# SerezD/vqvae-vqgan-pytorch-lightning

Measured on AMD Instinct MI355X. Metric: images/sec/node (256x256 bs=32/GPU) VQ-VAE train step, higher is better.
Workload: dtype bf16; 1 GPU; standard_vqvae cb=1024, 256x256 bs=32/GPU (encoder+VQ+decoder fwd/bwd + AdamW); yaml=example_confs/standard_vqvae.yaml, global_batch=32, parallelism=dp1, launch=hipGraph replay (fwd+bwd) + eager all-reduce + AdamW, deterministic=False

## Files before the change

### vqvae-vqgan-pytorch-lightning_amd/csrc/conv_mx.hip

```cpp
#include "conv_geom.h"
#include <stdlib.h>

namespace {
using vqkd::ConvGeom;
using vqkd::pack_bf16x2;
using vqkd::xcd_remap;

#ifndef VQK_MXABL
#define VQK_MXABL 0
#endif
#ifndef VQK_MX_RD
#define VQK_MX_RD 6
#endif
#ifndef VQK_MX_NT
#define VQK_MX_NT 2
#endif
#ifndef VQK_MX_HALO_AUX
#define VQK_MX_HALO_AUX 0
#endif
#ifndef VQK_MX_PRIO
#define VQK_MX_PRIO 0
#endif
#ifndef VQK_MX_PACE
#define VQK_MX_PACE 0
#endif
#ifndef VQK_MX_WL
#define VQK_MX_WL 0
#endif
#ifndef VQK_MX_JOUTER
#define VQK_MX_JOUTER 0
#endif
#ifndef VQK_MX_PIN
#define VQK_MX_PIN 1
#endif

#define SGB(mask, n) __builtin_amdgcn_sched_group_barrier(mask, n, 0)

__host__ __device__ constexpr int mx_tap_pix(bool s2, int tap, int twd, int hw2, int shp) {
    return s2 ? (((tap / 3) & 1) * 2 + ((tap % 3) & 1)) * shp + ((tap / 3) >> 1) * hw2 + ((tap % 3) >> 1)
              : (tap / twd) * hw2 + (tap % twd);
}

template <int TWLOG, bool POOL, int NTAP, int PIXELS = 256, int TAPW = 0, bool S2 = false>
__global__ __launch_bounds__(512, 2) void conv3x3_mx_kernel(const bf16_raw* __restrict__ x, const bf16_raw* __restrict__ wp,
                                                            const float* __restrict__ bias,
                                                            const bf16_raw* __restrict__ res, bf16_raw* __restrict__ y,
                                                            ConvGeom g) {
    constexpr int HM = NTAP == 1 ? 0 : 1;
    constexpr int PIX = PIXELS, TW = 1 << TWLOG, TH = PIX / TW;
    constexpr int HW2 = S2 ? TW + 1 : TW + 2 * HM;
    constexpr int SHP = (TH + 1) * (TW + 1);
    constexpr int HROWS = S2 ? 4 * SHP : (TH + 2 * HM) * HW2;
    constexpr int RS = 80;
    constexpr int PIECES = (HROWS * 5 + 63) / 64;
    constexpr int NBUF = S2 ? 2 : 3;
    constexpr int BUF = PIECES * 1024, STG = NBUF * BUF, SPITCH = 272, SCR = STG + PIX * SPITCH;
    constexpr int TQR = SCR + 1024;
    constexpr int TWD = TAPW ? TAPW : NTAP == 9 ? 3 : NTAP == 4 ? 2 : 1;
    constexpr int NI = VQK_MX_WL ? PIX / 32 : PIX / 64, NJ = VQK_MX_WL ? 1 : 2;
    constexpr int NQ = PIX / 16;
    static_assert(PIX == 256 || ((PIX == 128 || PIX == 64) && !POOL && NTAP == 9), "256-pixel tiles, or plain 128- / 64-pixel part tiles");
    constexpr int NPH = NTAP * 2;
    static_assert(NTAP == 9 || ((NTAP == 4 || NTAP == 2 || NTAP == 1) && !POOL), "3x3 taps, the 2x2 / 1x2 / 2x1 taps of a phase, or a 1x1 conv");
    static_assert(!S2 || (NTAP == 9 && !POOL && PIX == 128), "stride 2: 3x3 taps, 128-pixel tiles");
    static_assert(TAPW == 0 || (NTAP == 2 && (TAPW == 1 || TAPW == 2)), "TAPW names the orientation of a 2-tap window");
    constexpr int XS = (PIECES + 3) / 4;
    constexpr int OOB = (int)0x80000000;
    typedef bf16x8_t frag_t;
    typedef __attribute__((ext_vector_type(4))) unsigned int u32x4;
    typedef __attribute__((ext_vector_type(2))) unsigned int u32x2;
    extern __shared__ __attribute__((aligned(16))) char smem[];

    const int tid = threadIdx.x, lane = tid & 63;
    const int wave = __builtin_amdgcn_readfirstlane(tid >> 6);
    const int tiles_x = g.w >> TWLOG, tiles_y = g.h / TH;
    const int pmode = NTAP == 4 ? g.phase_mode : 0;
    const int total_tiles = g.n * tiles_y * tiles_x * g.tiles_n * (pmode == 1 ? 4 : 1);
    const int nch = g.cpt >> 2;
    const int nun = pmode == 2 ? 4 * nch : nch;
    const int grid = (int)gridDim.x, q8 = grid >> 3, r8 = grid & 7, xcd = (int)blockIdx.x & 7;
    const int cnt = q8 + (xcd < r8 ? 1 : 0);
    const int c0 = xcd < r8 ? xcd * (q8 + 1) : r8 * (q8 + 1) + (xcd - r8) * q8;
    const int vbid = c0 + ((int)blockIdx.x >> 3);
    if (vbid >= total_tiles) return;
    auto tile_of = [&](int k) -> int { const int j = k / cnt; return c0 + (k - j * cnt) + j * grid; };
    const int tqm = g.tq ? g.tq_mode : 0;
    volatile VQK_LDS int* const ring = (volatile VQK_LDS int*)(smem + TQR);
    auto next_id = [&](int j) -> int { return tqm ? __builtin_amdgcn_readfirstlane(ring[j & 7]) : vbid + j * grid; };
    const bool pro_sync = tqm == 2 || (tqm && nun < 4);

    struct TilePos { int img, py0, px0, nt, ph; };
    auto tile_pos = [&](int t) -> TilePos {
        TilePos tp;
        tp.nt = t % g.tiles_n; t /= g.tiles_n;
        tp.ph = 0;
        if (pmode == 1) { tp.ph = t & 3; t >>= 2; }
        const int txi = t % tiles_x; t /= tiles_x;
        const int tyi = t % tiles_y;
        tp.img = t / tiles_y; tp.py0 = tyi * TH; tp.px0 = txi * TW;
        return tp;
    };
    auto unit_barrier = [&]() { asm volatile("s_waitcnt lgkmcnt(0)\n\ts_barrier" ::: "memory"); };
    double* const gnws = (VQK_MXABL & 64) ? nullptr : g.gn_ws;
    unsigned long long* const dbg = (VQK_MXABL & 64) ? reinterpret_cast<unsigned long long*>(g.gn_ws) : nullptr;

    if (wave < 4) {
        if (VQK_MX_PRIO) __builtin_amdgcn_s_setprio(VQK_MX_PRIO);
        const int wm = VQK_MX_WL ? 0 : wave >> 1, wn = VQK_MX_WL ? wave : wave & 1;
        const int p = lane & 31, kg = lane >> 5;
        unsigned abase[NI], sbase[NI];
#pragma unroll
        for (int i = 0; i < NI; ++i) {
            int ty, tx;
            if (TWLOG == 5) { ty = wm * NI + i; tx = p; }
            else { ty = wm * 2 * NI + 2 * i + (p >> 4); tx = p & 15; }
            abase[i] = (unsigned)(((ty + (pmode ? 0 : g.tap_oy)) * HW2 + tx + (pmode ? 0 : g.tap_ox)) * RS + kg * 16);
            sbase[i] = (unsigned)(STG + (ty * TW + tx) * SPITCH + (wn * (32 * NJ) + 4 * kg) * 2);
        }
        const int lane16 = lane * 16;
        const int phase_bytes = (g.cout >> 5) * nch * (NPH * 1024);
        const __amdgpu_buffer_rsrc_t wsrd = __builtin_amdgcn_make_buffer_rsrc(
            const_cast<bf16_raw*>(wp), 0, phase_bytes * (pmode ? 4 : 1), 0x00020000);
        auto unit_ph = [&](int key, int c) -> int { return pmode == 2 ? c / nch : (key >> 16); };
        auto unit_w = [&](int key, int c, int j) -> int {
            const int ph = unit_ph(key, c), cc = pmode == 2 ? c - ph * nch : c;
            const int wph = (NTAP == 4 && g.phase_rev) ? 3 - ph : ph;
            return wph * phase_bytes + (((key & 0xffff) * 4 + wn * NJ + j) * nch + cc) * (NPH * 1024);
        };
        auto phase_off = [&](int ph) -> int {
            const int a = ph >> 1, b = ph & 1;
            return pmode == 1 ? (a * HW2 + b) * RS : pmode == 2 ? ((1 - a) * HW2 + (1 - b)) * RS : 0;
        };
        auto tile_nt = [&](int t) -> int {
            return (t % g.tiles_n) | (pmode == 1 ? ((t / g.tiles_n) & 3) << 16 : 0);
        };
        auto wload = [&](int soff) -> frag_t {
            return __builtin_bit_cast(frag_t, __builtin_amdgcn_raw_buffer_load_b128(wsrd, lane16, soff, 0));
        };

        constexpr int RD = NTAP == 9 ? VQK_MX_RD : NTAP == 4 ? 4 : 2;
        static_assert(NPH % RD == 0, "weight ring depth must divide the phases of a unit");
        f32x16 acc[NI][NJ];
        frag_t bw[RD][NJ];
        int wcur[NJ];
        if (pro_sync) unit_barrier();
        const int t_first = tqm == 2 ? __builtin_amdgcn_readfirstlane(ring[0]) : vbid;
        if (t_first >= total_tiles) return;
        int cur_nt = tile_nt(t_first);
#pragma unroll
        for (int j = 0; j < NJ; ++j) wcur[j] = unit_w(cur_nt, 0, j);
#pragma unroll
        for (int d = 0; d < RD; ++d)
#pragma unroll
            for (int j = 0; j < NJ; ++j) bw[d][j] = wload(wcur[j] + d * 1024);
        unit_barrier();

        int tj = 0, c = 0, bi = 0, t_next = 0;
        unsigned long long t_bar = 0, t_park = 0, n_units = 0, t_c0 = 0, t_cl = 0, t_top = 0;
        const unsigned long long t_begin = (VQK_MXABL & 64) ? __builtin_amdgcn_s_memtime() : 0;
        for (;;) {
            if (VQK_MXABL & 64) t_top = __builtin_amdgcn_s_memtime();
            if (c == nun - 2) t_next = next_id(tj + 1);
            const bool last_c = c == nun - 1, more = last_c && t_next < total_tiles;
            int nc = c + 1, nxt_nt = cur_nt;
            if (last_c) {
                if (more) { nc = 0; nxt_nt = tile_nt(t_next); }
                else nc = c;
            }
            int wnxt[NJ];
#pragma unroll
            for (int j = 0; j < NJ; ++j) wnxt[j] = unit_w(nxt_nt, nc, j);
            const char* lbase[NI];
#pragma unroll
            for (int i = 0; i < NI; ++i) lbase[i] = smem + bi * BUF + abase[i] + (NTAP == 4 ? phase_off(unit_ph(cur_nt, c)) : 0);

            frag_t a[2][NI];
#pragma unroll
            for (int i = 0; i < NI; ++i) a[0][i] = *reinterpret_cast<const frag_t*>(lbase[i]);
            __builtin_amdgcn_sched_barrier(0);
#pragma unroll
            for (int tap = 0; tap < NTAP; ++tap) {
                const int toff = mx_tap_pix(S2, tap, TWD, HW2, SHP) * RS;
#pragma unroll
                for (int ks = 0; ks < 2; ++ks) {
                    const bool reads = ks == 0 || tap < NTAP - 1;
                    const int ph = tap * 2 + ks;
                    if (ks == 0) {
#pragma unroll
                        for (int i = 0; i < NI; ++i) a[1][i] = *reinterpret_cast<const frag_t*>(lbase[i] + toff + 32);
                    } else if (tap < NTAP - 1) {
                        const int toff1 = mx_tap_pix(S2, tap + 1, TWD, HW2, SHP) * RS;
#pragma unroll
                        for (int i = 0; i < NI; ++i) a[0][i] = *reinterpret_cast<const frag_t*>(lbase[i] + toff1);
                    }
                    if (tap == 0 && ks == 0 && c == 0) {
                        const f32x16 zero = {0.f, 0.f, 0.f, 0.f, 0.f, 0.f, 0.f, 0.f, 0.f, 0.f, 0.f, 0.f, 0.f, 0.f, 0.f, 0.f};
#pragma unroll
                        for (int i = 0; i < NI; ++i)
#pragma unroll
                            for (int j = 0; j < NJ; ++j)
                                acc[i][j] = __builtin_amdgcn_mfma_f32_32x32x16_bf16(bw[ph % RD][j], a[ks][i], zero, 0, 0, 0);
                    } else if (VQK_MX_JOUTER) {
#pragma unroll
                        for (int j = 0; j < NJ; ++j)
#pragma unroll
                            for (int i = 0; i < NI; ++i)
                                acc[i][j] = __builtin_amdgcn_mfma_f32_32x32x16_bf16(bw[ph % RD][j], a[ks][i], acc[i][j], 0, 0, 0);
                    } else {
#pragma unroll
                        for (int i = 0; i < NI; ++i)
#pragma unroll
                            for (int j = 0; j < NJ; ++j)
                                acc[i][j] = __builtin_amdgcn_mfma_f32_32x32x16_bf16(bw[ph % RD][j], a[ks][i], acc[i][j], 0, 0, 0);
                    }
#pragma unroll
                    for (int j = 0; j < NJ; ++j) {
                        const int soff = (ph + RD >= NPH) ? wnxt[j] + (ph + RD - NPH) * 1024 : wcur[j] + (ph + RD) * 1024;
                        bw[ph % RD][j] = wload(((VQK_MXABL & 32) && g.n > 0 && wm == 1) ? (soff & 1023) : soff);
                    }
                    if (VQK_MX_PIN) {
                        if (reads) {
#pragma unroll
                            for (int i = 0; i < NI; ++i) { SGB(0x008, 1); SGB(0x100, 1); }
                            if constexpr (NI * NJ - NI > 0) SGB(0x008, NI * NJ - NI);
                        } else {
                            SGB(0x008, NI * NJ);
                        }
                        SGB(0x020, NJ);
                    }
                    __builtin_amdgcn_sched_barrier(0);
                }
            }
            const unsigned long long t_a = (VQK_MXABL & 64) ? __builtin_amdgcn_s_memtime() : 0;
            if (VQK_MXABL & 64) { if (c == 0) t_c0 += t_a - t_top; if (c == nun - 1) t_cl += t_a - t_top; }
            if (c == nun - 1 && !((VQK_MXABL & 4) && g.n > 0)) {
#pragma unroll
                for (int i = 0; i < NI; ++i)
#pragma unroll
                    for (int j = 0; j < NJ; ++j)
#pragma unroll
                        for (int rq = 0; rq < 4; ++rq) {
                            const u32x2 o = {pack_bf16x2(acc[i][j][4 * rq], acc[i][j][4 * rq + 1]),
                                             pack_bf16x2(acc[i][j][4 * rq + 2], acc[i][j][4 * rq + 3])};
                            *reinterpret_cast<u32x2*>(smem + sbase[i] + (j * 32 + 8 * rq) * 2) = o;
                        }
            }
            if (VQK_MXABL & 64) {
                asm volatile("s_waitcnt lgkmcnt(0)" ::: "memory");
                const unsigned long long t_b = __builtin_amdgcn_s_memtime();
                unit_barrier();
                const unsigned long long t_c = __builtin_amdgcn_s_memtime();
                t_park += t_b - t_a; t_bar += t_c - t_b; ++n_units;
            } else
            unit_barrier();
            if (last_c) { if (!more) break; ++tj; }
            cur_nt = nxt_nt; c = nc;
            bi = bi == NBUF - 1 ? 0 : bi + 1;
#pragma unroll
            for (int j = 0; j < NJ; ++j) wcur[j] = wnxt[j];
        }
        if ((VQK_MXABL & 64) && dbg && lane == 0) {
            unsigned long long* o = dbg + ((int64_t)blockIdx.x * 4 + wave) * 8;
            o[0] = __builtin_amdgcn_s_memtime() - t_begin; o[1] = t_bar; o[2] = t_park; o[3] = n_units;
            o[4] = t_c0; o[5] = t_cl; o[6] = (unsigned long long)nun; o[7] = 0;
        }
        return;
    }

    const int xt = tid - 256, xw = wave - 4;
    const __amdgpu_buffer_rsrc_t xsrd = __builtin_amdgcn_make_buffer_rsrc(
        const_cast<bf16_raw*>(x), 0, (int)((int64_t)g.n * g.h_in * g.w_in * g.cin * 2), 0x00020000);
    const int out_bytes = (int)((int64_t)g.n * g.dst_h * g.dst_w * g.cout * 2);
    const __amdgpu_buffer_rsrc_t rsrd = __builtin_amdgcn_make_buffer_rsrc(const_cast<bf16_raw*>(res), 0, res ? out_bytes : 0, 0x00020000);
    const __amdgpu_buffer_rsrc_t ysrd = __builtin_amdgcn_make_buffer_rsrc(y, 0, out_bytes >> (POOL ? 2 : 0), 0x00020000);

    int rel[XS], flg[XS];
#pragma unroll
    for (int sl = 0; sl < XS; ++sl) {
        const int s = (xw + 4 * sl) * 64 + lane;
        const int hp = s / 5, cp = s - hp * 5;
        if constexpr (S2) {
            const int sh = hp / SHP, q = hp - sh * SHP;
            const int hy = q / HW2, hx = q - hy * HW2, pa = sh >> 1, pb = sh & 1;
            rel[sl] = (((2 * hy + pa) * g.w_in + 2 * hx + pb) * g.cin + cp * 8) * 2;
            flg[sl] = (cp == 4 || hp >= HROWS || (pa && hy == TH) || (pb && hx == TW)) ? 16 : 0;
        } else {
            const int hy = hp / HW2, hx = hp - hy * HW2;
            rel[sl] = (((((hy - HM) * g.src_s) >> g.ups) * g.w_in + (((hx - HM) * g.src_s) >> g.ups)) * g.cin + cp * 8) * 2;
            flg[sl] = (HM && hy == 0 ? 1 : 0) | (HM && hy == TH + 1 ? 2 : 0) | (HM && hx == 0 ? 4 : 0) | (HM && hx == TW + 1 ? 8 : 0) |
                      ((cp == 4 || hp >= HROWS) ? 16 : 0);
        }
    }
    auto issue_halo = [&](const TilePos& tp, int cu, int bufi) {
        const int uph = pmode == 2 ? cu / nch : 0, c = pmode == 2 ? cu - uph * nch : cu;
        const int sa = pmode == 2 ? (uph >> 1) : g.src_a, sb = pmode == 2 ? (uph & 1) : g.src_b;
        const int base = (((tp.img * g.h_in + ((tp.py0 * g.src_s + sa) >> g.ups)) * g.w_in + ((tp.px0 * g.src_s + sb) >> g.ups)) * g.cin + c * 32) * 2;
        const int tb = S2 ? 16 : ((tp.py0 == 0 ? 1 : 0) | (tp.py0 + TH == g.h ? 2 : 0) | (tp.px0 == 0 ? 4 : 0) | (tp.px0 + TW == g.w ? 8 : 0) | 16);
#pragma unroll
        for (int sl = 0; sl < XS; ++sl) {
            if (xw + 4 * sl < PIECES) {
                const int off = (flg[sl] & tb) ? OOB : base + rel[sl];
                __builtin_amdgcn_raw_ptr_buffer_load_lds(
                    xsrd, (VQK_LDS void*)(smem + bufi * BUF + (xw + 4 * sl) * 1024), 16,
                    (VQK_MXABL & 8) ? (off & 0x8003fff0) : off, 0, 0, VQK_MX_HALO_AUX);
            }
        }
    };
    auto unpack8 = [&](const u32x4& r, float (&v)[8]) {
#pragma unroll
        for (int e = 0; e < 4; ++e) { v[2 * e] = __uint_as_float(r[e] << 16); v[2 * e + 1] = __uint_as_float(r[e] & 0xffff0000u); }
    };
    auto pack8 = [&](const float (&v)[8]) -> u32x4 {
        const u32x4 o = {pack_bf16x2(v[0], v[1]), pack_bf16x2(v[2], v[3]), pack_bf16x2(v[4], v[5]), pack_bf16x2(v[6], v[7])};
        return o;
    };
    const int slot = xt & 15;
    constexpr int NP = POOL ? 4 : NQ;
    constexpr int NR = NQ;
    struct OutPos { int pix0, ppix0, co, img, tile; };
    auto out_pos = [&](const TilePos& tp) -> OutPos {
        OutPos o;
        o.tile = (tp.py0 / TH) * tiles_x + (tp.px0 >> TWLOG) + (pmode == 1 ? tp.ph * tiles_y * tiles_x : 0);
        const int da = pmode == 1 ? (tp.ph >> 1) : g.dst_a, db = pmode == 1 ? (tp.ph & 1) : g.dst_b;
        o.pix0 = (tp.img * g.dst_h + tp.py0 * g.dst_s + da) * g.dst_w + tp.px0 * g.dst_s + db;
        o.ppix0 = (tp.img * (g.h >> 1) + (tp.py0 >> 1)) * (g.w >> 1) + (tp.px0 >> 1);
        o.co = tp.nt * 128 + slot * 8;
        o.img = tp.img;
        return o;
    };
    auto res_off = [&](const OutPos& o, int k) -> int {
        int ty, tx;
        if constexpr (!POOL) { const int pp = k * 16 + (xt >> 4); ty = pp >> TWLOG; tx = pp & (TW - 1); }
        else { const int opp = (k >> 2) * 16 + (xt >> 4); ty = 2 * (opp >> (TWLOG - 1)) + ((k >> 1) & 1); tx = 2 * (opp & (TW / 2 - 1)) + (k & 1); }
        return ((o.pix0 + (ty * g.dst_w + tx) * g.dst_s) * g.cout + o.co) * 2;
    };
    auto load_res = [&](const OutPos& o, u32x4 (&rv)[NR]) {
#pragma unroll
        for (int k = 0; k < NR; ++k)
            rv[k] = __builtin_bit_cast(u32x4, __builtin_amdgcn_raw_buffer_load_b128(rsrd, res_off(o, k), 0, 0));
    };
    int stat_idx = -1;
    auto flush_stats = [&]() {
        if (xw == 0) {
            float v = 0.f;
#pragma unroll
            for (int k = 0; k < 4; ++k) v += *reinterpret_cast<const float*>(smem + SCR + (k * 64 + lane) * 4);
            if (g.gn_part_nblk) {
                const int span = g.gn_cpg >> 3;
                if (span >= 2) v += __shfl_xor(v, 1, 64);
                if (span >= 4) v += __shfl_xor(v, 2, 64);
                if (stat_idx >= 0 && (span < 2 || (lane & (span - 1)) == 0)) gnws[stat_idx] = (double)v;
            } else if (stat_idx >= 0) {
                atomicAdd(gnws + stat_idx, (double)v);
            }
        }
    };
    float ga = 0.f, qa = 0.f, gb = 0.f, qb = 0.f;
    auto drain = [&](const OutPos& o, const u32x4 (&rv)[NR], int k0, int k1, bool first, bool last) {
        if (first) { ga = 0.f; qa = 0.f; gb = 0.f; qb = 0.f; }
        float bv[8] = {0.f, 0.f, 0.f, 0.f, 0.f, 0.f, 0.f, 0.f};
        if (bias) {
            const f32x4 b0 = *reinterpret_cast<const f32x4*>(bias + o.co), b1 = *reinterpret_cast<const f32x4*>(bias + o.co + 4);
#pragma unroll
            for (int e = 0; e < 4; ++e) { bv[e] = b0[e]; bv[4 + e] = b1[e]; }
        }
        const bool want_stats = gnws != nullptr;
        const unsigned ones2 = 0x3f803f80u;
        auto tally = [&](const u32x4& o) {
            const unsigned d0 = o[0], d1 = o[1], d2 = o[2], d3 = o[3];
            asm("v_dot2c_f32_bf16 %0, %4, %8\n\tv_dot2c_f32_bf16 %1, %4, %4\n\tv_dot2c_f32_bf16 %2, %6, %8\n\t"
                "v_dot2c_f32_bf16 %3, %6, %6\n\tv_dot2c_f32_bf16 %0, %5, %8\n\tv_dot2c_f32_bf16 %1, %5, %5\n\t"
                "v_dot2c_f32_bf16 %2, %7, %8\n\tv_dot2c_f32_bf16 %3, %7, %7\n\ts_nop 0"
                : "+v"(ga), "+v"(qa), "+v"(gb), "+v"(qb) : "v"(d0), "v"(d1), "v"(d2), "v"(d3), "v"(ones2));
        };
        auto settle = [&]() { asm volatile("s_nop 3" : "+v"(ga), "+v"(qa), "+v"(gb), "+v"(qb)); };
        u32x4 t[NQ];
        if constexpr (!POOL) {
#pragma unroll
            for (int k = 0; k < NQ; ++k) {
                if (k < k0 || k >= k1) continue;
                t[k] = *reinterpret_cast<const u32x4*>(smem + STG + (k * 16 + (xt >> 4)) * SPITCH + slot * 16);
            }
        } else {
#pragma unroll
            for (int k = 0; k < NQ; ++k) {
                if ((k >> 2) < k0 || (k >> 2) >= k1) continue;
                const int opp = (k >> 2) * 16 + (xt >> 4);
                const int ty = 2 * (opp >> (TWLOG - 1)) + ((k >> 1) & 1), tx = 2 * (opp & (TW / 2 - 1)) + (k & 1);
                t[k] = *reinterpret_cast<const u32x4*>(smem + STG + (ty * TW + tx) * SPITCH + slot * 16);
            }
        }
        __builtin_amdgcn_sched_barrier(0);
        if constexpr (!POOL) {
            if (!bias && !res && g.act == 0 && g.acc_scale == 1.0f && g.out_gain == 1.0f) {
#pragma unroll
                for (int k = 0; k < NP; ++k) {
                    if (k < k0 || k >= k1) continue;
                    __builtin_amdgcn_raw_buffer_store_b128(t[k], ysrd, res_off(o, k), 0, VQK_MX_NT);
                    if (want_stats) tally(t[k]);
                }
            } else {
                const bool general = g.act != 0 || g.acc_scale != 1.0f || g.out_gain != 1.0f;
                float abl_b[8] = {0.f, 0.f, 0.f, 0.f, 0.f, 0.f, 0.f, 0.f}, abl_g[8] = {0.f, 0.f, 0.f, 0.f, 0.f, 0.f, 0.f, 0.f};
#pragma unroll
                for (int k = 0; k < NP; ++k) {
                    if (k < k0 || k >= k1) continue;
                    float f[8], r[8];
                    unpack8(t[k], f);
                    unpack8(rv[k], r);
                    if ((VQK_MXABL & 16) && g.n > 0) {
#pragma unroll
                        for (int e = 0; e < 8; ++e) {
                            const float xh = __fmaf_rn(r[e], 1.3f, -0.13f);
                            const float u = __fmaf_rn(xh, 1.1f, 0.05f);
                            const float sg = __frcp_rn(1.0f + __expf(-u));
                            const float t = f[e] * (sg * (1.0f + u * (1.0f - sg)));
                            abl_b[e] += t;
                            abl_g[e] = __fmaf_rn(t, xh, abl_g[e]);
                        }
                    }
                    if (general) {
#pragma unroll
                        for (int e = 0; e < 8; ++e) {
                            float v = __fmaf_rn(f[e], g.acc_scale, bv[e]);
                            v = g.act == 2 ? fmaxf(v, 0.0f) : g.act == 3 ? fmaxf(v, 0.2f * v) : v;
                            f[e] = __fmaf_rn(v, g.out_gain, r[e]);
                        }
                    } else {
#pragma unroll
                        for (int e = 0; e < 8; ++e) f[e] = f[e] + bv[e] + r[e];
                    }
                    const u32x4 ov = pack8(f);
                    __builtin_amdgcn_raw_buffer_store_b128(ov, ysrd, res_off(o, k), 0, VQK_MX_NT);
                    if (want_stats) tally(ov);
                }
                if ((VQK_MXABL & 16) && g.n > 0) {
#pragma unroll
                    for (int e = 0; e < 8; ++e) { ga += abl_b[e]; qa += abl_g[e]; }
                }
            }
        } else {
#pragma unroll
            for (int k = 0; k < NP; ++k) {
                if (k < k0 || k >= k1) continue;
                const int opp = k * 16 + (xt >> 4);
                const int oty = opp >> (TWLOG - 1), otx = opp & (TW / 2 - 1);
                float s[8] = {0.f, 0.f, 0.f, 0.f, 0.f, 0.f, 0.f, 0.f};
#pragma unroll
                for (int d = 0; d < 4; ++d) {
                    float f[8], r[8];
                    unpack8(t[4 * k + d], f);
                    unpack8(rv[4 * k + d], r);
#pragma unroll
                    for (int e = 0; e < 8; ++e) s[e] += f[e] + r[e];
                }
#pragma unroll
                for (int e = 0; e < 8; ++e) s[e] = (s[e] + 4.0f * bv[e]) * g.pool_scale;
                const u32x4 ov = pack8(s);
                __builtin_amdgcn_raw_buffer_store_b128(ov, ysrd, ((o.ppix0 + oty * (g.w >> 1) + otx) * g.cout + o.co) * 2, 0, VQK_MX_NT);
                if (want_stats) tally(ov);
            }
        }
        if (want_stats && last) {
            settle();
            const bool split = g.gn_cpg == 4;
            if (!split) { ga += gb; qa += qb; }
            ga += __shfl_xor(ga, 16, 64); ga += __shfl_xor(ga, 32, 64);
            qa += __shfl_xor(qa, 16, 64); qa += __shfl_xor(qa, 32, 64);
            if (split) {
                gb += __shfl_xor(gb, 16, 64); gb += __shfl_xor(gb, 32, 64);
                qb += __shfl_xor(qb, 16, 64); qb += __shfl_xor(qb, 32, 64);
            }
            const int q = (xt >> 4) & 3;
            const float val = q == 0 ? ga : q == 1 ? qa : q == 2 ? gb : qb;
            *reinterpret_cast<float*>(smem + SCR + (xw * 64 + lane) * 4) = val;
            const int grp = (o.co + (q >> 1) * 4) / g.gn_cpg;
            const int gslot = o.img * (g.cout / g.gn_cpg) + grp;
            stat_idx = (split || q < 2) ? ((g.gn_part_nblk ? gslot * g.gn_part_nblk + g.gn_part_base + o.tile : gslot) * 2 + (q & 1)) : -1;
        }
    };

    int nissued = tqm == 2 ? 0 : 1, exhausted = 0, pend = 0, fv = 0;
    const int qbase = tqm == 2 ? 0 : cnt;
    auto fetch_issue = [&]() {
        if (lane == 0) fv = __hip_atomic_fetch_add(g.tq + xcd, 1, __ATOMIC_RELAXED, __HIP_MEMORY_SCOPE_AGENT);
        pend = 1;
    };
    auto fetch_land = [&]() {
        const int t = tile_of(__builtin_amdgcn_readfirstlane(fv) + qbase);
        if (lane == 0) ring[nissued & 7] = t;
        ++nissued; pend = 0;
        if (t >= total_tiles) exhausted = 1;
    };
    auto census = [&]() {
        if (tqm && xw == 0 && lane == 0) {
            const int old = __hip_atomic_fetch_add(g.tq + 8, 1, __ATOMIC_RELAXED, __HIP_MEMORY_SCOPE_AGENT);
            if (old == grid - 1) {
#pragma unroll
                for (int i = 0; i < 9; ++i) __hip_atomic_exchange(g.tq + i, 0, __ATOMIC_RELAXED, __HIP_MEMORY_SCOPE_AGENT);
            }
        }
    };
    if (tqm && xw == 0) {
        const int need = 3 / nun;
        while (nissued <= need && !exhausted) { fetch_issue(); fetch_land(); }
    }
    if (pro_sync) unit_barrier();
    const int t_first = tqm == 2 ? __builtin_amdgcn_readfirstlane(ring[0]) : vbid;
    if (t_first >= total_tiles) { census(); return; }

    int ltj = 0, lc = 0, lbuf = 0, lvalid = 1, lnew = 0;
    TilePos ltp = tile_pos(t_first);
    auto look = [&]() {
        if (lnew) {
            lnew = 0;
            if (lvalid) {
                const int t = next_id(ltj);
                lvalid = t < total_tiles;
                if (lvalid) ltp = tile_pos(t);
            }
        }
    };
    auto bump = [&]() {
        if (++lc == nun) { lc = 0; ++ltj; lnew = 1; }
        lbuf = lbuf == NBUF - 1 ? 0 : lbuf + 1;
    };
    issue_halo(ltp, lc, lbuf); bump();
    if constexpr (NBUF == 3) { look(); if (lvalid) issue_halo(ltp, lc, lbuf); bump(); }
    int tj = 0, c = 0;
    TilePos cur = tile_pos(t_first);
    OutPos done = out_pos(cur);
    int fu = 4 % nun, ford = 4 / nun;
    bool pending = false, flush = false;
    int dk = 0;
    u32x4 rv[NR];
#pragma unroll
    for (int k = 0; k < NR; ++k) rv[k] = u32x4{0u, 0u, 0u, 0u};
    asm volatile("s_waitcnt vmcnt(0)" ::: "memory");
    unit_barrier();

    for (;;) {
        asm volatile("s_waitcnt vmcnt(0)" ::: "memory");
        if (tqm && xw == 0) {
            if (pend) fetch_land();
            if (!exhausted && ford >= nissued) fetch_issue();
        }
        if (++fu == nun) { fu = 0; ++ford; }
        if constexpr (NBUF == 2) {
            look();
            if (lvalid) issue_halo(ltp, lc, lbuf);
            bump();
        }
        if (flush) { flush_stats(); flush = false; }
        if (pending && !((VQK_MXABL & 2) && g.n > 0)) {
            const int per = (VQK_MX_PACE && nun > 2) ? (NP + nun - 2) / (nun - 1) : NP;
            const int k1 = dk + per < NP ? dk + per : NP;
            drain(done, rv, dk, k1, dk == 0, k1 == NP);
            dk = k1;
            if (dk == NP) { pending = false; dk = 0; flush = gnws != nullptr; }
        }
        const bool last_c = c == nun - 1;
        int t_next = 0;
        if (last_c) {
            pending = true;
            done = out_pos(cur);
            if (res) load_res(done, rv);
            t_next = next_id(tj + 1);
        }
        if constexpr (NBUF == 3) {
            look();
            if (lvalid && !((VQK_MXABL & 1) && g.n > 0)) issue_halo(ltp, lc, lbuf);
            bump();
        } else {
            asm volatile("s_waitcnt vmcnt(0)" ::: "memory");
        }
        unit_barrier();
        if (last_c) {
            if (t_next >= total_tiles) break;
            c = 0; ++tj; cur = tile_pos(t_next);
        } else {
            ++c;
        }
    }
    if (flush) flush_stats();
    if (pending) {
        asm volatile("s_waitcnt vmcnt(0)" ::: "memory");
        drain(done, rv, dk, NP, dk == 0, true);
        if (gnws) {
            unit_barrier();
            flush_stats();
        }
    }
    census();
}

}

namespace vqkd {

namespace {
template <auto Kern>
int mx_launch(dim3 grid, int lds, hipStream_t st, const void* x, const void* w, const float* bias, const void* res, void* y,
              const ConvGeom& g) {
    static const hipError_t attr = hipFuncSetAttribute((const void*)Kern, hipFuncAttributeMaxDynamicSharedMemorySize, lds);
    if (attr != hipSuccess) return VQK_ERR_LAUNCH;
    hipLaunchKernelGGL(Kern, grid, dim3(512), lds, st, (const bf16_raw*)x, (const bf16_raw*)w, bias, (const bf16_raw*)res,
                       (bf16_raw*)y, g);
    return hipGetLastError() == hipSuccess ? VQK_OK : VQK_ERR_LAUNCH;
}

int device_cus() {
    static const int cus = [] {
        int dev = 0, n = 0;
        if (hipGetDevice(&dev) != hipSuccess ||
            hipDeviceGetAttribute(&n, hipDeviceAttributeMultiprocessorCount, dev) != hipSuccess || n <= 0) n = 256;
        return n;
    }();
    return cus;
}
}

int launch_conv3x3_mx(const void* x, const void* w, const float* bias, const void* res, void* y, const void* zeros,
                      const ConvGeom& g_in, int twlog, hipStream_t st) {
    (void)zeros;
    ConvGeom g = g_in;
    if (!g.dst_h) { g.dst_h = g.h * g.dst_s; g.dst_w = g.w * g.dst_s; }
    const int half_on = VQK_TUNE("MX_HALF", 1);
    const int half_hw = VQK_TUNE("MX_HALF_HW", 256);
    const bool half = half_on && g.h * g.w <= half_hw && !g.pool && g.ntap == 9 && (twlog == 4 ? (g.h % 8) == 0 : (g.h % 4) == 0);
    const int qmode = VQK_TUNE("MX_QUARTER", 1);
    const bool quarter = half && qmode && (g.tiles_n <= 2 || qmode >= 2) && (twlog == 4 ? (g.h % 4) == 0 : (g.h % 2) == 0);
    const int th = (quarter ? 64 : half ? 128 : 256) >> twlog;
    const int total = g.n * (g.h / th) * (g.w >> twlog) * g.tiles_n * ((g.ntap == 4 && g.phase_mode == 1) ? 4 : 1);
    int cus = device_cus() - VQK_TUNE("COMM_CUS", 0);
    if (cus < 1) cus = 1;
    const dim3 grid((unsigned)(total < cus ? total : cus));
    const int tqm = VQK_TUNE("TILE_QUEUE", 0);
    const DetState& tqs = tile_queue_state();
    auto set_queue = [&](int tiles, int blocks) {
        const bool on = tqm > 0 && tqs.ws != nullptr && tqs.bytes >= 64 && tiles > blocks && (g.cpt >> 2) >= 2;
        g.tq = on ? reinterpret_cast<int*>(tqs.ws) : nullptr;
        g.tq_mode = on ? (tqm >= 2 ? 2 : 1) : 0;
    };
    set_queue(total, (int)grid.x);
    constexpr int TQB = 64;
    constexpr int lds5 = 3 * (((256 / 32 + 2) * 34 * 5 + 63) / 64) * 1024 + 256 * 272 + 1024 + TQB;
    constexpr int lds4 = 3 * (((256 / 16 + 2) * 18 * 5 + 63) / 64) * 1024 + 256 * 272 + 1024 + TQB;
    constexpr int lds4h = 3 * (((128 / 16 + 2) * 18 * 5 + 63) / 64) * 1024 + 128 * 272 + 1024 + TQB;
    constexpr int lds5h = 3 * (((128 / 32 + 2) * 34 * 5 + 63) / 64) * 1024 + 128 * 272 + 1024 + TQB;
#define MXL(K, L) return mx_launch<K>(grid, L, st, x, w, bias, res, y, g)
    constexpr int lds4q = 3 * (((64 / 16 + 2) * 18 * 5 + 63) / 64) * 1024 + 64 * 272 + 1024 + TQB;
    constexpr int lds5q = 3 * (((64 / 32 + 2) * 34 * 5 + 63) / 64) * 1024 + 64 * 272 + 1024 + TQB;
    if (g.s2) {
        constexpr int lds5s = 2 * ((4 * (128 / 32 + 1) * 33 * 5 + 63) / 64) * 1024 + 128 * 272 + 1024 + TQB;
        constexpr int lds4s = 2 * ((4 * (128 / 16 + 1) * 17 * 5 + 63) / 64) * 1024 + 128 * 272 + 1024 + TQB;
        if (g.pool || g.ntap != 9 || (twlog == 4 ? (g.h % 8) : (g.h % 4)) != 0) return VQK_ERR_ARG;
        const int tot2 = g.n * (g.h / (128 >> twlog)) * (g.w >> twlog) * g.tiles_n;
        const dim3 grid2((unsigned)(tot2 < cus ? tot2 : cus));
        set_queue(tot2, (int)grid2.x);
        if (twlog == 5) return mx_launch<conv3x3_mx_kernel<5, false, 9, 128, 0, true>>(grid2, lds5s, st, x, w, bias, res, y, g);
        return mx_launch<conv3x3_mx_kernel<4, false, 9, 128, 0, true>>(grid2, lds4s, st, x, w, bias, res, y, g);
    }
    if (g.ntap == 2) {
        if (g.pool) return VQK_ERR_ARG;
        if (g.tapw == 2) { if (twlog == 5) MXL((conv3x3_mx_kernel<5, false, 2, 256, 2>), lds5); else MXL((conv3x3_mx_kernel<4, false, 2, 256, 2>), lds4); }
        if (g.tapw == 1) { if (twlog == 5) MXL((conv3x3_mx_kernel<5, false, 2, 256, 1>), lds5); else MXL((conv3x3_mx_kernel<4, false, 2, 256, 1>), lds4); }
        return VQK_ERR_ARG;
    }
    if (quarter) {
        if (twlog == 5) MXL((conv3x3_mx_kernel<5, false, 9, 64>), lds5q); else MXL((conv3x3_mx_kernel<4, false, 9, 64>), lds4q);
    } else if (half) {
        if (twlog == 5) MXL((conv3x3_mx_kernel<5, false, 9, 128>), lds5h); else MXL((conv3x3_mx_kernel<4, false, 9, 128>), lds4h);
    } else if (g.ntap == 4) {
        if (g.pool) return VQK_ERR_ARG;
        if (twlog == 5) MXL((conv3x3_mx_kernel<5, false, 4>), lds5); else MXL((conv3x3_mx_kernel<4, false, 4>), lds4);
    } else if (g.ntap == 1) {
        if (g.pool) return VQK_ERR_ARG;
        constexpr int lds1 = 3 * ((256 * 5 + 63) / 64) * 1024 + 256 * 272 + 1024 + TQB;
        if (twlog == 5) MXL((conv3x3_mx_kernel<5, false, 1>), lds1); else MXL((conv3x3_mx_kernel<4, false, 1>), lds1);
    } else if (twlog == 5) {
        if (g.pool) MXL((conv3x3_mx_kernel<5, true, 9>), lds5); else MXL((conv3x3_mx_kernel<5, false, 9>), lds5);
    } else {
        if (g.pool) MXL((conv3x3_mx_kernel<4, true, 9>), lds4); else MXL((conv3x3_mx_kernel<4, false, 9>), lds4);
    }
#undef MXL
}

}
```

Measured before the change: 1132 images/sec.

## Use 16x16x32 bf16 MFMA path in implicit-GEMM 3x3 conv kernel

Adds a default-on variant of the main conv loop that issues mfma_f32_16x16x32_bf16 instead of the 32x32 instructions. It splits each pixel tile into two 16-row halves with separate accumulators, remaps the lane-to-pixel/K layout and the weight-fragment load offsets, and uses a shallower weight ring indexed per tap. The epilogue is rewritten to match the 16x16 output layout. The aim is better MFMA throughput or latency hiding on MI355X. The cost is a changed register footprint and fragment layout that must match the packed weight format exactly.

```diff
diff --git a/vqvae-vqgan-pytorch-lightning_amd/csrc/conv_mx.hip b/vqvae-vqgan-pytorch-lightning_amd/csrc/conv_mx.hip
--- a/vqvae-vqgan-pytorch-lightning_amd/csrc/conv_mx.hip
+++ b/vqvae-vqgan-pytorch-lightning_amd/csrc/conv_mx.hip
@@ -32,6 +32,9 @@
 #endif
 #ifndef VQK_MX_PIN
 #define VQK_MX_PIN 1
+#endif
+#ifndef VQK_MX_MFMA16
+#define VQK_MX_MFMA16 1
 #endif
 
 #define SGB(mask, n) __builtin_amdgcn_sched_group_barrier(mask, n, 0)
@@ -65,6 +68,8 @@
     static_assert(!S2 || (NTAP == 9 && !POOL && PIX == 128), "stride 2: 3x3 taps, 128-pixel tiles");
     static_assert(TAPW == 0 || (NTAP == 2 && (TAPW == 1 || TAPW == 2)), "TAPW names the orientation of a 2-tap window");
     constexpr int XS = (PIECES + 3) / 4;
+    constexpr bool M16 = VQK_MX_MFMA16 && !VQK_MX_WL && !S2 && (NTAP == 9 || NTAP == 4);
+    constexpr int HOFF = (TWLOG == 5 ? 16 : HW2) * RS;
     constexpr int OOB = (int)0x80000000;
     typedef bf16x8_t frag_t;
     typedef __attribute__((ext_vector_type(4))) unsigned int u32x4;
@@ -107,7 +112,7 @@
     if (wave < 4) {
         if (VQK_MX_PRIO) __builtin_amdgcn_s_setprio(VQK_MX_PRIO);
         const int wm = VQK_MX_WL ? 0 : wave >> 1, wn = VQK_MX_WL ? wave : wave & 1;
-        const int p = lane & 31, kg = lane >> 5;
+        const int p = M16 ? lane & 15 : lane & 31, kg = M16 ? lane >> 4 : lane >> 5;
         unsigned abase[NI], sbase[NI];
 #pragma unroll
         for (int i = 0; i < NI; ++i) {
@@ -117,7 +122,11 @@
             abase[i] = (unsigned)(((ty + (pmode ? 0 : g.tap_oy)) * HW2 + tx + (pmode ? 0 : g.tap_ox)) * RS + kg * 16);
             sbase[i] = (unsigned)(STG + (ty * TW + tx) * SPITCH + (wn * (32 * NJ) + 4 * kg) * 2);
         }
-        const int lane16 = lane * 16;
+        auto sbase16 = [&](int i) -> unsigned {
+            const int ty = TWLOG == 5 ? wm * NI + i : wm * 2 * NI + 2 * i, tx = p;
+            return (unsigned)(STG + (ty * TW + tx) * SPITCH + (wn * 64 + 4 * kg) * 2);
+        };
+        const int lane16 = M16 ? (lane >> 5) * 1024 + (((lane >> 4) & 1) * 32 + (lane & 15)) * 16 : lane * 16;
         const int phase_bytes = (g.cout >> 5) * nch * (NPH * 1024);
         const __amdgpu_buffer_rsrc_t wsrd = __builtin_amdgcn_make_buffer_rsrc(
             const_cast<bf16_raw*>(wp), 0, phase_bytes * (pmode ? 4 : 1), 0x00020000);
@@ -140,8 +149,19 @@
 
         constexpr int RD = NTAP == 9 ? VQK_MX_RD : NTAP == 4 ? 4 : 2;
         static_assert(NPH % RD == 0, "weight ring depth must divide the phases of a unit");
+        constexpr int RDT = NTAP == 9 ? 3 : 2;
         f32x16 acc[NI][NJ];
         frag_t bw[RD][NJ];
+        f32x4 acc16[2][NI][2 * NJ];
+        if constexpr (M16) {
+#pragma unroll
+            for (int h = 0; h < 2; ++h)
+#pragma unroll
+                for (int i = 0; i < NI; ++i)
+#pragma unroll
+                    for (int jj = 0; jj < 2 * NJ; ++jj) acc16[h][i][jj] = f32x4{0.f, 0.f, 0.f, 0.f};
+        }
+        frag_t bw16[RDT][2 * NJ];
         int wcur[NJ];
         if (pro_sync) unit_barrier();
         const int t_first = tqm == 2 ? __builtin_amdgcn_readfirstlane(ring[0]) : vbid;
@@ -149,10 +169,17 @@
         int cur_nt = tile_nt(t_first);
 #pragma unroll
         for (int j = 0; j < NJ; ++j) wcur[j] = unit_w(cur_nt, 0, j);
-#pragma unroll
-        for (int d = 0; d < RD; ++d)
-#pragma unroll
-            for (int j = 0; j < NJ; ++j) bw[d][j] = wload(wcur[j] + d * 1024);
+        if constexpr (M16) {
+#pragma unroll
+            for (int d = 0; d < RDT; ++d)
+#pragma unroll
+                for (int jj = 0; jj < 2 * NJ; ++jj) bw16[d][jj] = wload(wcur[jj >> 1] + d * 2048 + (jj & 1) * 256);
+        } else {
+#pragma unroll
+            for (int d = 0; d < RD; ++d)
+#pragma unroll
+                for (int j = 0; j < NJ; ++j) bw[d][j] = wload(wcur[j] + d * 1024);
+        }
         unit_barrier();
 
         int tj = 0, c = 0, bi = 0, t_next = 0;
@@ -178,6 +205,49 @@
 #pragma unroll
             for (int i = 0; i < NI; ++i) a[0][i] = *reinterpret_cast<const frag_t*>(lbase[i]);
             __builtin_amdgcn_sched_barrier(0);
+            if constexpr (M16) {
+#pragma unroll
+            for (int tap = 0; tap < NTAP; ++tap) {
+                const int toff = mx_tap_pix(S2, tap, TWD, HW2, SHP) * RS;
+                const int ws = tap % RDT;
+#pragma unroll
+                for (int h = 0; h < 2; ++h) {
+                    const bool reads = h == 0 || tap < NTAP - 1;
+                    if (h == 0) {
+#pragma unroll
+                        for (int i = 0; i < NI; ++i) a[1][i] = *reinterpret_cast<const frag_t*>(lbase[i] + toff + HOFF);
+                    } else if (tap < NTAP - 1) {
+                        const int toff1 = mx_tap_pix(S2, tap + 1, TWD, HW2, SHP) * RS;
+#pragma unroll
+                        for (int i = 0; i < NI; ++i) a[0][i] = *reinterpret_cast<const frag_t*>(lbase[i] + toff1);
+                    }
+#pragma unroll
+                    for (int i = 0; i < NI; ++i)
+#pragma unroll
+                        for (int jj = 0; jj < 2 * NJ; ++jj)
+                            acc16[h][i][jj] = __builtin_amdgcn_mfma_f32_16x16x32_bf16(bw16[ws][jj], a[h][i], acc16[h][i][jj], 0, 0, 0);
+                    if (h == 1) {
+                        const int tt = tap + RDT;
+#pragma unroll
+                        for (int jj = 0; jj < 2 * NJ; ++jj) {
+                            const int soff = tt >= NTAP ? wnxt[jj >> 1] + (tt - NTAP) * 2048 : wcur[jj >> 1] + tt * 2048;
+                            bw16[ws][jj] = wload(soff + (jj & 1) * 256);
+                        }
+                    }
+                    if (VQK_MX_PIN) {
+                        if (reads) {
+#pragma unroll
+                            for (int i = 0; i < NI; ++i) { SGB(0x008, 1); SGB(0x100, 1); }
+                            SGB(0x008, NI * 2 * NJ - NI);
+                        } else {
+                            SGB(0x008, NI * 2 * NJ);
+                        }
+                        if (h == 1) SGB(0x020, 2 * NJ);
+                    }
+                    __builtin_amdgcn_sched_barrier(0);
+                }
+            }
+            } else {
 #pragma unroll
             for (int tap = 0; tap < NTAP; ++tap) {
                 const int toff = mx_tap_pix(S2, tap, TWD, HW2, SHP) * RS;
@@ -231,9 +301,23 @@
                     __builtin_amdgcn_sched_barrier(0);
                 }
             }
+            }
             const unsigned long long t_a = (VQK_MXABL & 64) ? __builtin_amdgcn_s_memtime() : 0;
             if (VQK_MXABL & 64) { if (c == 0) t_c0 += t_a - t_top; if (c == nun - 1) t_cl += t_a - t_top; }
             if (c == nun - 1 && !((VQK_MXABL & 4) && g.n > 0)) {
+              if constexpr (M16) {
+#pragma unroll
+                for (int i = 0; i < NI; ++i)
+#pragma unroll
+                    for (int h = 0; h < 2; ++h)
+#pragma unroll
+                        for (int jj = 0; jj < 2 * NJ; ++jj) {
+                            const u32x2 o = {pack_bf16x2(acc16[h][i][jj][0], acc16[h][i][jj][1]),
+                                             pack_bf16x2(acc16[h][i][jj][2], acc16[h][i][jj][3])};
+                            *reinterpret_cast<u32x2*>(smem + sbase16(i) + h * 16 * SPITCH + jj * 32) = o;
+                            acc16[h][i][jj] = f32x4{0.f, 0.f, 0.f, 0.f};
+                        }
+              } else {
 #pragma unroll
                 for (int i = 0; i < NI; ++i)
 #pragma unroll
@@ -244,6 +328,7 @@
                                              pack_bf16x2(acc[i][j][4 * rq + 2], acc[i][j][4 * rq + 3])};
                             *reinterpret_cast<u32x2*>(smem + sbase[i] + (j * 32 + 8 * rq) * 2) = o;
                         }
+              }
             }
             if (VQK_MXABL & 64) {
                 asm volatile("s_waitcnt lgkmcnt(0)" ::: "memory");
```

After: 1138 images/sec, median of 6. Within noise of the previous version (+0.5%).
